# panagiotou23/model-predictive-control

Hardware: AMD Instinct MI355X
Metric: MPC solves/sec, bicycle model N=20 nx=4 nu=2, batch=65536; 1/2/4/8 GPU (higher is better)
Workload: dtype f64

## Files before the change

### include/mpc_hip.h

```cpp
#ifndef MPC_HIP_H
#define MPC_HIP_H
#include <stdint.h>

#ifdef __cplusplus
extern "C" {
#endif

enum { MPC_MODEL_KINEMATIC = 0,
       MPC_MODEL_PACEJKA = 1 };
enum { MPC_WRAP_FLOOR = 0, MPC_WRAP_FMOD = 1, MPC_WRAP_IEEE = 2 };
enum { MPC_CONSTR_NONE = 0,
       MPC_CONSTR_STATE_SQ = 1,
       MPC_CONSTR_LANE = 2,
       MPC_CONSTR_DISCS = 3 };
enum { MPC_ST_UNKNOWN = 0, MPC_ST_CONVERGED = 1, MPC_ST_MAXTIME = 2, MPC_ST_MAXITER = 3,
       MPC_ST_NOTFINITE = 4, MPC_ST_NOPROGRESS = 5, MPC_ST_INTERRUPTED = 6 };
enum { MPC_OK = 0, MPC_E_ARG = -1, MPC_E_HIP = -2, MPC_E_ALLOC = -3, MPC_E_LIMIT = -4 };

#define MPC_NSTATS 8
#define MPC_MAX_N 64
#define MPC_NREC 64

typedef struct mpc_config {
    int32_t model;
// ... 83 lines not shown

int mpc_rhs(mpc_handle *h, int B, const double *x, const double *u, double *dx, void *stream);

int mpc_rollout(mpc_handle *h, int B, int Nsim, const double *x0, const double *U, double *X,
                void *stream);

int mpc_centerline_blocks(mpc_handle *h, const double *cl, int C, void *stream);
int mpc_set_nearest_blocks(mpc_handle *h, int on);

int mpc_stage_errors(mpc_handle *h, int B, const double *pose, const double *cl,
                     const int32_t *cl_index, double *err, int32_t *idx, void *stream);

int mpc_stage_cost(mpc_handle *h, int B, const double *x, const double *u, const double *cl,
                   const int32_t *cl_index, double *out, void *stream);

int mpc_eval_cost_grad(mpc_handle *h, int B, const double *x0, const double *cl,
                       const int32_t *cl_index, const double *U, const double *y,
                       const double *Sigma, double *psi, double *grad, double *yhat, void *stream);

int mpc_eval_cost_grad_wave(mpc_handle *h, int B, const double *x0, const double *cl,
                            const int32_t *cl_index, const double *U, const double *y,
                            const double *Sigma, double *psi, double *grad, double *yhat, void *stream);

int mpc_prox_step(mpc_handle *h, int B, const double *x, const double *grad, const double *gamma,
                  double *xhat, double *p, double *out, void *stream);

int mpc_lbfgs_apply(mpc_handle *h, int B, const double *S, const double *Y, const int32_t *idx,
                    const int32_t *full, const double *mask, double *q, int32_t *ok, void *stream);

int mpc_solve_batch(mpc_handle *h, int B, const double *x0, const double *cl,
                    const int32_t *cl_index, double *U, double *lambda, double *stats,
                    void *stream);

int mpc_solve_batch_async(mpc_handle *h, int B, const double *x0, const double *cl,
                          const int32_t *cl_index, double *U, double *lambda, double *stats,
                          void *stream);
int mpc_solve_wait(mpc_handle *h);

int mpc_closed_loop(mpc_handle *h, int B, int T, int shift, double *x, const double *cl,
                    const int32_t *cl_index, double *U, double *lambda, double *traj_x,
                    double *traj_u, int32_t *fail_count, double *stats, void *stream);

int mpc_solve_active(mpc_handle *h, int B, const int32_t *active, const double *x0, const double *cl,
                     const int32_t *cl_index, double *U, double *lambda, double *stats, int32_t *n_active,
                     void *stream);

// ... 62 lines not shown
```

### model_predictive_control_amd/_lib.py

```python
import ctypes as C
import os
import subprocess

def _default_hw_queues():
    if "GPU_MAX_HW_QUEUES" in os.environ:
        return
    try:
        import torch
        if torch.cuda.is_initialized():
            return
    except Exception:
        pass
    os.environ["GPU_MAX_HW_QUEUES"] = "16"


_default_hw_queues()

_HERE = os.path.dirname(os.path.abspath(__file__))
LIB_PATH = os.environ.get("MPC_LIB_PATH", os.path.join(_HERE, "libmpc_hip.so"))
_SRC = [os.path.join(_HERE, "csrc", f) for f in ("mpc_api.hip", "mpc_handle.hpp", "mpc_launch.hpp", "mpc_rounds.hpp",
                                                  "mpc_aux.hpp", "mpc_eval.hpp", "mpc_solver.hpp", "mpc_device.hpp",
                                                  "mpc_game.hpp", "mpc_solo.hpp", "mpc_event.hpp", "mpc_step_body.hpp",
                                                  "mpc_track.hpp", "mpc_obstacles.hpp", "mpc_traffic.hpp")]
_HDR = os.path.join(os.path.dirname(_HERE), "include", "mpc_hip.h")

MODEL_KINEMATIC, MODEL_PACEJKA = 0, 1
WRAP_FLOOR, WRAP_FMOD, WRAP_IEEE = 0, 1, 2
CONSTR_NONE, CONSTR_STATE_SQ, CONSTR_LANE, CONSTR_DISCS = 0, 1, 2, 3
NSTATS = 8
ST_CONVERGED = 1

EXPORTS = [
    "mpc_default_config", "mpc_nx", "mpc_m", "mpc_create", "mpc_destroy", "mpc_last_error",
    "mpc_rhs", "mpc_rollout", "mpc_stage_errors", "mpc_stage_cost", "mpc_eval_cost_grad", "mpc_prox_step",
    "mpc_lbfgs_apply", "mpc_solve_batch", "mpc_solve_batch_async", "mpc_solve_wait", "mpc_closed_loop", "mpc_last_solve_info",
    "mpc_last_solve_info2", "mpc_math_probe", "mpc_set_groups", "mpc_last_kernel_ms", "mpc_lane_payoff",
    "mpc_set_profile", "mpc_last_speculation", "mpc_last_kernel_profile", "mpc_set_solo_max",
    "mpc_eval_cost_grad_wave", "mpc_centerline_blocks", "mpc_set_nearest_blocks", "mpc_set_memo",
    "mpc_set_round_limit", "mpc_stream_concurrency", "mpc_last_solo_ms",
    "mpc_set_poll_timeout", "mpc_debug_spin", "mpc_debug_records", "mpc_debug_record_names", "mpc_source_hash",
    "mpc_last_lookahead", "mpc_step_lds_plan", "mpc_default_params", "mpc_set_agent_params",
    "mpc_solve_active", "mpc_trigger_eval", "mpc_closed_loop_event",
    "mpc_default_bounds", "mpc_set_agent_bounds",
    "mpc_default_constraints", "mpc_set_agent_constraints",
    "mpc_default_discs", "mpc_set_agent_discs", "mpc_discs_from_plans",
    "mpc_default_rates", "mpc_set_agent_rates",
    "mpc_default_fields", "mpc_set_agent_fields", "mpc_fields_from_plans", "mpc_closed_loop_traffic_field",
    "mpc_opponents_from_plans", "mpc_closed_loop_traffic",
    "mpc_obstacles_select", "mpc_discs_from_obstacles", "mpc_fields_from_obstacles", "mpc_closed_loop_obstacles",
    "mpc_track_init", "mpc_track_windows", "mpc_track_locate", "mpc_track_select", "mpc_closed_loop_track",
]
NREC = 64
NPARAM = 31
NBOUND = 4
NCONSTR = 19
NRATE = 4
NFIELD = 2
NFSRC = 8
NDISC = 2
SCENE_MAX = 64
CONSTR_FIELDS = {"g_off": (0, 6), "D_lb": (6, 6), "D_ub": (12, 6), "lane_halfwidth": (18, 1)}
# ... 55 lines not shown
def load():
    global _lib
    if _lib is not None:
        return _lib
    if not os.path.exists(LIB_PATH):
        raise RuntimeError(
            f"{LIB_PATH} is missing: run `python -c 'import __graft_entry__ as g; g.build()'` "
            "(the MPC hot path has no CPU fallback)")
    L = C.CDLL(LIB_PATH)
    vp, ci = C.c_void_p, C.c_int
    cp = C.POINTER(MpcConfig)
    L.mpc_default_config.argtypes = [cp, ci, ci]
    L.mpc_nx.argtypes = [cp]
    L.mpc_m.argtypes = [cp]
    L.mpc_create.argtypes = [cp, ci, C.POINTER(vp)]
    L.mpc_destroy.argtypes = [vp]
    L.mpc_last_error.restype = C.c_char_p
    L.mpc_rhs.argtypes = [vp, ci, vp, vp, vp, vp]
    L.mpc_rollout.argtypes = [vp, ci, ci, vp, vp, vp, vp]
    L.mpc_stage_errors.argtypes = [vp, ci, vp, vp, vp, vp, vp, vp]
    L.mpc_stage_cost.argtypes = [vp, ci, vp, vp, vp, vp, vp, vp]
    L.mpc_eval_cost_grad.argtypes = [vp, ci, vp, vp, vp, vp, vp, vp, vp, vp, vp, vp]
    L.mpc_eval_cost_grad_wave.argtypes = [vp, ci, vp, vp, vp, vp, vp, vp, vp, vp, vp, vp]
    L.mpc_prox_step.argtypes = [vp, ci, vp, vp, vp, vp, vp, vp, vp]
    L.mpc_lbfgs_apply.argtypes = [vp, ci, vp, vp, vp, vp, vp, vp, vp, vp]
    L.mpc_solve_batch.argtypes = [vp, ci, vp, vp, vp, vp, vp, vp, vp]
    L.mpc_solve_batch_async.argtypes = [vp, ci, vp, vp, vp, vp, vp, vp, vp]
    L.mpc_solve_wait.argtypes = [vp]
    L.mpc_closed_loop.argtypes = [vp, ci, ci, ci, vp, vp, vp, vp, vp, vp, vp, vp, vp, vp]
    L.mpc_solve_active.argtypes = [vp, ci, vp, vp, vp, vp, vp, vp, vp, C.POINTER(C.c_int32), vp]
    L.mpc_trigger_eval.argtypes = [vp, ci, vp, vp, vp, C.POINTER(C.c_double), C.c_double, ci, vp, vp, vp]
    L.mpc_closed_loop_event.argtypes = [vp, ci, ci, ci, C.POINTER(C.c_double), C.c_double, ci, vp, vp, vp, vp, vp, vp,
                                        vp, vp, vp, vp, vp, vp, vp, vp]
    tp = C.POINTER(MpcTrack)
    L.mpc_track_init.argtypes = [tp, cp, ci, ci, ci, ci, ci]
    L.mpc_track_windows.argtypes = [vp, tp, vp, vp, vp]
    L.mpc_track_locate.argtypes = [vp, tp, ci, vp, vp, vp, vp, vp]
    L.mpc_track_select.argtypes = [vp, tp, ci, vp, vp, vp, vp, vp, vp]
    L.mpc_closed_loop_track.argtypes = L.mpc_closed_loop_event.argtypes + [tp, vp]
    L.mpc_last_solve_info.argtypes = [vp, C.POINTER(C.c_int64), C.POINTER(C.c_int64),
                                      C.POINTER(C.c_int64), C.POINTER(C.c_double),
                                      C.POINTER(C.c_double)]
    L.mpc_last_solve_info2.argtypes = [vp, C.POINTER(C.c_double), C.POINTER(C.c_int64)]
    L.mpc_last_speculation.argtypes = [vp, C.POINTER(C.c_int64), C.POINTER(C.c_int64)]
    L.mpc_last_lookahead.argtypes = [vp, C.POINTER(C.c_int64), C.POINTER(C.c_int64)]
    L.mpc_default_params.argtypes = [cp, C.POINTER(C.c_double)]
# ... 289 lines not shown
```

### model_predictive_control_amd/csrc/mpc_api.hip

```cpp
#include "mpc_rounds.hpp"
#include "mpc_track.hpp"
#include "mpc_obstacles.hpp"

extern "C" const char *mpc_last_error(void) { return g_err.c_str(); }
#ifndef MPC_SOURCE_SHA256
#define MPC_SOURCE_SHA256 "unknown"
#endif
extern "C" const char *mpc_source_hash(void) { return MPC_SOURCE_SHA256; }

extern "C" int mpc_default_config(mpc_config *c, int model, int N)
{
    if (!c || N < 1 || N > MPC_MAX_N || (model != MPC_MODEL_KINEMATIC && model != MPC_MODEL_PACEJKA))
        return fail(MPC_E_ARG, "mpc_default_config: bad model or horizon");
    std::memset(c, 0, sizeof(*c));
    c->model = model; c->N = N;
    c->S = 100;
    c->nfe = 4;
    c->wrap_mode = MPC_WRAP_FLOOR;
    c->lbfgs_memory = N;
    c->max_iter = 1000;
    c->max_outer = 1000;
    c->hess_heuristic = 15;
    c->max_no_progress = 10;
    c->Ts = 0.05;
// ... 412 lines not shown
    hipLaunchKernelGGL(math_probe_kernel, grid_for(n, 256), dim3(256), 0, (hipStream_t)stream, n, op, a, b, out);
    HIPCHK(hipGetLastError());
    return MPC_OK;
}

extern "C" int mpc_stage_cost(mpc_handle *h, int B, const double *x, const double *u, const double *cl,
                              const int32_t *cl_index, double *out, void *stream)
{
    int rc = check_common(h, B, "mpc_stage_cost"); if (rc) return rc;
    if (B == 0) return MPC_OK;
    if (!x || !u || !cl || !out) return fail(MPC_E_ARG, "mpc_stage_cost: null buffer");
    rc = check_tables(h, B, "mpc_stage_cost", READS_PARAMS); if (rc) return rc;
    hipStream_t s = (hipStream_t)stream;
    with_model_table(h, h->params().idx, [&](auto MODEL, auto PA, auto... pt) {
        hipLaunchKernelGGL((stage_cost_kernel<MODEL(), PA(), decltype(pt)...>), grid_for(B, 64), dim3(64), 0, s,
                           h->dc, B, x, u, cl, cl_index, out, pt...);
    });
    HIPCHK(hipGetLastError());
    return MPC_OK;
}

static int eval_cost_grad(mpc_handle *h, int B, const double *x0, const double *cl, const int32_t *cl_index,
                          const double *U, const double *y, const double *Sigma, double *psi, double *grad,
                          double *yhat, void *stream, bool wave_path)
{
    int rc = check_common(h, B, "mpc_eval_cost_grad"); if (rc) return rc;
    if (B == 0) return MPC_OK;
    if (!x0 || !cl || !U || !psi) return fail(MPC_E_ARG, "mpc_eval_cost_grad: null buffer");
    const DevCfg &c = h->dc;
    if (c.m && (!y || !Sigma)) return fail(MPC_E_ARG, "mpc_eval_cost_grad: y and Sigma are required when m > 0");
    rc = check_tables(h, B, "mpc_eval_cost_grad", READS_PARAMS | READS_CONSTR | READS_DISCS | READS_RATES | READS_FIELDS, true); if (rc) return rc;
    rc = reserve(h, B); if (rc) return rc;
    hipStream_t s = (hipStream_t)stream;
    WorkspaceHost w = h->ws;
    w.cl = cl; w.cl_index = cl_index; w.x0 = x0; w.near = near_for(h, cl);
    w.xe = const_cast<double *>(U); w.ge = grad ? grad : h->ws.ws_ge;
    w.y = const_cast<double *>(y); w.Sig = c.m ? const_cast<double *>(Sigma) : h->ws.ws_Sig;
    w.yhe = (yhat && c.m) ? yhat : h->ws.ws_yhe;
    w.psi_direct = psi;
    w.ptab = h->params().table; w.pidx = h->params().idx;
    w.ctab = h->tab[TAB_CONSTR].table; w.cidx = h->tab[TAB_CONSTR].idx;
    w.dtab = h->tab[TAB_DISCS].table; w.didx = h->tab[TAB_DISCS].idx;
    w.rtab = h->tab[TAB_RATES].table; w.ridx = h->tab[TAB_RATES].idx;
    w.ftab = h->tab[TAB_FIELDS].table; w.fidx = h->tab[TAB_FIELDS].idx;
    if (wave_path) launch_solo_eval(h, w, s, grad ? 1 : 0);
    else launch_eval(h, w, s, nullptr, nullptr, grad ? B : 0, grad ? 0 : B);
    HIPCHK(hipGetLastError());
    return MPC_OK;
}
extern "C" int mpc_eval_cost_grad(mpc_handle *h, int B, const double *x0, const double *cl, const int32_t *cl_index, const double *U,
                                  const double *y, const double *Sigma, double *psi, double *grad, double *yhat, void *stream)
{
    return eval_cost_grad(h, B, x0, cl, cl_index, U, y, Sigma, psi, grad, yhat, stream, false);
}
extern "C" int mpc_eval_cost_grad_wave(mpc_handle *h, int B, const double *x0, const double *cl, const int32_t *cl_index, const double *U,
                                       const double *y, const double *Sigma, double *psi, double *grad, double *yhat, void *stream)
{
    return eval_cost_grad(h, B, x0, cl, cl_index, U, y, Sigma, psi, grad, yhat, stream, true);
}

extern "C" int mpc_prox_step(mpc_handle *h, int B, const double *x, const double *grad, const double *gamma,
                             double *xhat, double *p, double *out, void *stream)
{
    int rc = check_common(h, B, "mpc_prox_step"); if (rc) return rc;
    if (B == 0) return MPC_OK;
    if (!x || !grad || !gamma || !out) return fail(MPC_E_ARG, "mpc_prox_step: null buffer");
    rc = check_tables(h, B, "mpc_prox_step", READS_BOX); if (rc) return rc;
    if (const BoundTable &box = h->tab[TAB_BOX]; box.table)
        hipLaunchKernelGGL(prox_box_kernel, grid_for(B, 64), dim3(64), 0, (hipStream_t)stream, h->dc, B, x, grad, gamma, xhat, p, out,
                           BoxTab{box.table, box.idx});
    else
        hipLaunchKernelGGL(prox_kernel, grid_for(B, 64), dim3(64), 0, (hipStream_t)stream, h->dc, B, x, grad, gamma, xhat, p, out);
    HIPCHK(hipGetLastError());
    return MPC_OK;
}

extern "C" int mpc_lbfgs_apply(mpc_handle *h, int B, const double *S, const double *Y, const int32_t *idx,
                               const int32_t *full, const double *mask, double *q, int32_t *ok, void *stream)
{
    int rc = check_common(h, B, "mpc_lbfgs_apply"); if (rc) return rc;
    if (B == 0) return MPC_OK;
// ... 803 lines not shown
```

### model_predictive_control_amd/csrc/mpc_eval.hpp

```cpp
#pragma once
#include "mpc_solver.hpp"

#ifndef MPC_K1B_WAVES_PAC
#define MPC_K1B_WAVES_PAC 1
#endif
#ifndef MPC_QUAD_WAVES
#define MPC_QUAD_WAVES 2
#endif

namespace mpc {

struct SlotMap {
    int nG, nC, gpad, nblk_g, nblk;
    __device__ SlotMap(const int *counts, int nG_imm, int nC_imm)
    {
        nG = counts ? counts[0] : nG_imm;
        nC = counts ? counts[1] : nC_imm;
        gpad = (nG + 63) & ~63;
        nblk_g = gpad >> 6;
        nblk = nblk_g + ((nC + 63) >> 6);
    }
};

template <int MODEL, bool PA = false>
// ... 307 lines not shown
            double gx, gy;
            kin_gen_rk(c, uk, g ? cv[p] : 0.0, kr);
            kin_gen_increment(c, uk, g ? cph[p] : 0.0, g ? cv[p] : 0.0, kr, gx, gy);
            dx[p] = g ? gx : dx[p]; dy[p] = g ? gy : dy[p];
        }
    }
    double px = x0[0], py = x0[1], epx = 0.0, epy = 0.0;
#pragma unroll
    for (int p = 0; p < PASS; p++) {
        const int k0 = 16 * p, k1 = N < 16 * (p + 1) ? N : 16 * (p + 1);
        for (int k = k0; k < k1; k++) {
#pragma clang fp contract(off)
#pragma unroll
            for (int j = 0; j < 4; j++) {
                px = px + rdlane(dx[p], (4 * k + j) & 63);
                py = py + rdlane(dy[p], (4 * k + j) & 63);
            }
            if (lane == k) { epx = px; epy = py; }
        }
    }
    if (stage_lane) { put(lane + 1, 0, epx); put(lane + 1, 1, epy); put(lane + 1, 2, eph); put(lane + 1, 3, ev); }
}

template <bool PA = false>
__global__ void __launch_bounds__(256)
rollout_wide_kernel(const DevCfg c, const WsArg<PA> w, const int *__restrict__ lists,
                    const int *__restrict__ counts)
{
    const SlotMap sm(counts, 0, 0);
    const int lane = threadIdx.x & 63, wv = threadIdx.x >> 6;
    const int uslot = blockIdx.x * 4 + wv;
    if (uslot >= sm.nblk * 64) return;
    const bool is_g = uslot < sm.gpad;
    const int kslot = is_g ? uslot : uslot - sm.gpad;
    const bool active = kslot < (is_g ? sm.nG : sm.nC);
    const int raw = active ? (is_g ? lists : lists + w.Ls)[kslot] : -1;
    if (lane == 0) w.agent_of[uslot] = raw;
    if (!active) return;
    const int a = raw & AGENT_MASK;
    const int N = c.N, n = c.n;
    const size_t St = (size_t)w.St;
    const double *__restrict__ row = ((raw & CH2_BIT) ? w.xe2 : w.xe) + (size_t)a * n;
    const bool stage_lane = lane < N;
    const double d = stage_lane ? row[2 * lane] : 0.0, dl = stage_lane ? row[2 * lane + 1] : 0.0;
    if (stage_lane) {
        w.useq[(size_t)(2 * lane) * St + uslot] = d;
// ... 382 lines not shown
```

### model_predictive_control_amd/csrc/mpc_solo.hpp

```cpp
#pragma once
#include "mpc_eval.hpp"

namespace mpc {

constexpr int SOLO_WAVES = 1;

__host__ __device__ inline bool solo_wide(int model, int nfe) { return model == KIN && nfe == 4; }
__host__ __device__ inline bool solo_dual(int model, int nfe, int N) { return !solo_wide(model, nfe) && N <= 32; }

constexpr int LA_SLOTS = 4, LA_LANES = 16, LA_ENTRIES = 8;
__host__ __device__ inline bool solo_lookahead(int model, int nfe, int N, int m, int no_la)
{
    return model == PAC && !no_la && m == 0 && N <= LA_LANES && solo_dual(model, nfe, N);
}
struct LaSlot { const double *in; double *grad; double *psi; int live, is_g; };
__host__ __device__ inline size_t la_lds_doubles(int n) { return (size_t)LA_ENTRIES * (2 * n + 2) + LA_SLOTS * 4 + 8; }

template <int MODEL> __host__ __device__ inline size_t solo_lds_doubles(int nfe, int N, int n, int M, bool hist, bool la = false)
{
    constexpr int NX = ModelDim<MODEL>::NX, JS = JacRec<MODEL>::SIZE;
    const size_t per = (size_t)(N + 1) * NX + (size_t)(JS + 1) * N;
    return (hist ? (size_t)2 * M * n : 0) + (la ? LA_SLOTS : solo_dual(MODEL, nfe, N) ? 2 : 1) * per + (la ? la_lds_doubles(n) : 0);
}

#if MPC_DEV_STAMP == 5
struct SoloClk { long long roll = 0, recs = 0, adj = 0; };
#define SOLO_CLK_ARG , SoloClk &clk
#define SOLO_CLK(field, t) do { const long long now_ = __builtin_amdgcn_s_memrealtime(); clk.field += now_ - t; t = now_; } while (0)
#else
#define SOLO_CLK_ARG
#define SOLO_CLK(field, t) do { } while (0)
#endif
template <int MODEL, class... DS>
__device__ __forceinline__ void solo_eval(const DevCfg &c, const Workspace &w, int a, int lane, int req,
                                          double *traj, double *rec SOLO_CLK_ARG, const DS &...ds)
{
#if MPC_DEV_STAMP == 5
    long long tclk = __builtin_amdgcn_s_memrealtime();
#endif
    constexpr int NX = ModelDim<MODEL>::NX, JS = JacRec<MODEL>::SIZE;
    const int N = c.N, n = c.n;
    const bool wide = solo_wide(MODEL, c.nfe), dual = solo_dual(MODEL, c.nfe, N);
    const int half = dual ? lane >> 5 : 0, hl = dual ? lane & 31 : lane;
    const bool ch2 = half == 1;
    const bool live = !ch2 || (req & REQ_SPEC) != 0;
    const bool is_g = ch2 || (req & REQ_GRAD) != 0;
    const double *__restrict__ row = (ch2 ? w.xe2 : w.xe) + (size_t)a * n;
    const bool stage_lane = live && hl < N;
    const double d = stage_lane ? row[2 * hl] : 0.0, dl = stage_lane ? row[2 * hl + 1] : 0.0;
    double *const tj = traj + (size_t)half * ((size_t)(N + 1) * NX);
    double *const rc = rec + (size_t)half * ((size_t)(JS + 1) * N);
    double x0[NX];
#pragma unroll
    for (int i = 0; i < NX; i++) x0[i] = w.x0[(size_t)a * NX + i];
    if constexpr (MODEL == KIN) {
        if (wide) kin_wide_rollout(c, x0, d, dl, lane, [=](int k, int i, double v) { tj[k * 4 + i] = v; });
    }
    if constexpr (MODEL == PAC) {
        if (hl < 4 && live) {
            double x[NX];
#pragma unroll
            for (int i = 0; i < NX; i++) { x[i] = x0[i]; if (hl == 0) tj[i] = x0[i]; }
            for (int k = 0; k < N; k++) {
                StageInput<PAC> u;
                prep_input(c, row[2 * k], row[2 * k + 1], u);
                stage_forward_quad(c, u, x, hl);
                if (hl == 0) {
#pragma unroll
                    for (int i = 0; i < NX; i++) tj[(k + 1) * NX + i] = x[i];
                }
            }
        }
    } else if (!wide && hl == 0 && live) {
        double x[NX];
#pragma unroll
        for (int i = 0; i < NX; i++) { x[i] = x0[i]; tj[i] = x0[i]; }
        for (int k = 0; k < N; k++) {
            StageInput<MODEL> u;
            prep_input(c, row[2 * k], row[2 * k + 1], u);
// ... 11 lines not shown
        const double *__restrict__ clp = w.cl_index ? w.cl + (size_t)w.cl_index[a] * 2 * (size_t)c.S : w.cl;
        double *const r = rc + hl;
        const auto put = [=](int f, double v) { r[f * N] = v; };
        if (is_g) stage_sens_record<MODEL>(c, xs, xe, d, dl, put);
        Geom g;
        stage_geom(c, w, clp, w.cl_index ? w.cl_index[a] : 0, xe[0], xe[1], g);
        constexpr bool DA = has_tab<DiscTab, DS...>, RA = has_tab<RateTab, DS...>, FA = has_tab<FieldTab, DS...>;
        if constexpr (FA)
            stage_record<MODEL>(c, w, a, ch2, is_g, hl, xs, xe, d, dl, g, put, stage_rate_uniform(pack_get<RateTab>(ds...), a, hl, N, row),
                                stage_field_uniform(pack_get<FieldTab>(ds...), a, hl, N));
        else if constexpr (DA && RA)
            stage_record<MODEL>(c, w, a, ch2, is_g, hl, xs, xe, d, dl, g, put, stage_discs_uniform(pack_get<DiscTab>(ds...), a, hl, N),
                                stage_rate_uniform(pack_get<RateTab>(ds...), a, hl, N, row));
        else if constexpr (RA)
            stage_record<MODEL>(c, w, a, ch2, is_g, hl, xs, xe, d, dl, g, put, stage_rate_uniform(pack_get<RateTab>(ds...), a, hl, N, row));
        else if constexpr (DA) stage_record<MODEL>(c, w, a, ch2, is_g, hl, xs, xe, d, dl, g, put, stage_discs_uniform(ds..., a, hl, N));
        else
        stage_record<MODEL>(c, w, a, ch2, is_g, hl, xs, xe, d, dl, g, put);
    }
    __builtin_amdgcn_wave_barrier();
    SOLO_CLK(recs, tclk);
    if constexpr (MODEL == KIN) {
        if (hl < 4 && live) {
            double *psi_out = w.psi_direct ? w.psi_direct + a : !ch2 ? w.rec + (size_t)a * REC + R_PSIE : nullptr;
            adjoint_rec_quad_kin(c, is_g, hl, [=](int k, int f) { return rc[f * N + k]; }, psi_out,
                                 (ch2 ? w.ge2 : w.ge) + (size_t)a * n);
        }
    } else if (hl == 0 && live) adjoint_rec<MODEL>(c, w, a, ch2, is_g, [=](int k, int f) { return rc[f * N + k]; });
    SOLO_CLK(adj, tclk);
}

__device__ __forceinline__ void solo_eval_la(const DevCfg &c, const Workspace &w, int a, int lane, const LaSlot *slots,
                                             double *traj, double *rec)
{
    constexpr int NX = ModelDim<PAC>::NX, JS = JacRec<PAC>::SIZE;
    const int N = c.N;
    const int sl = lane >> 4, hl = lane & 15;
    const LaSlot d = slots[sl];
    const bool live = d.live != 0, is_g = d.is_g != 0;
    const double *__restrict__ row = d.in;
    const bool stage_lane = live && hl < N;
    const double dv = stage_lane ? row[2 * hl] : 0.0, dl = stage_lane ? row[2 * hl + 1] : 0.0;
    double *const tj = traj + (size_t)sl * ((size_t)(N + 1) * NX);
    double *const rc = rec + (size_t)sl * ((size_t)(JS + 1) * N);
    double x0[NX];
#pragma unroll
    for (int i = 0; i < NX; i++) x0[i] = w.x0[(size_t)a * NX + i];
// ... 50 lines not shown
{
    const int a = blockIdx.x * blockDim.x + threadIdx.x;
    const bool on = a < w.B && rec_int_of(w.rec[(size_t)a * REC + R_PHASE]) != PH_DONE;
    const unsigned long long bal = __ballot(on);
    const int lane = threadIdx.x & 63;
    int base = 0;
    if (lane == 0 && bal != 0ull) base = atomicAdd(&ctr[1], __popcll(bal));
    base = __builtin_amdgcn_readfirstlane(base);
    if (on) list[base + __popcll(bal & ((1ull << lane) - 1ull))] = a;
}

template <int MODEL, bool PA = false, class... CT>
__global__ void __launch_bounds__(64, 1) solo_eval_kernel(const DevCfg c_, const WsArg<PA> w, int want_grad, CT... ct)
{
    static_assert(sizeof...(CT) == 0 || PA, "the constraint form exists in the per-agent-parameter form alone");
    extern __shared__ double s_solo[];
    DevCfg cm_;
    if constexpr (PA) { cm_ = c_; agent_cfg_uniform(cm_, w.ptab, w.pidx, blockIdx.x); }
    constexpr bool DA = has_tab<DiscTab, CT...> || has_tab<RateTab, CT...>;
    if constexpr (has_tab<ConTab, CT...>) agent_con_uniform(cm_, ct..., blockIdx.x);
    const DevCfg &c = PA ? cm_ : c_;
    double *traj = s_solo;
    double *rec = traj + (size_t)(c.N + 1) * ModelDim<MODEL>::NX;
#if MPC_DEV_STAMP == 5
    SoloClk clk;
    if constexpr (DA) solo_eval<MODEL>(c, w, blockIdx.x, threadIdx.x, want_grad ? REQ_GRAD : REQ_COST, traj, rec, clk, ct...);
    else
    solo_eval<MODEL>(c, w, blockIdx.x, threadIdx.x, want_grad ? REQ_GRAD : REQ_COST, traj, rec, clk);
#else
    if constexpr (DA) solo_eval<MODEL>(c, w, blockIdx.x, threadIdx.x, want_grad ? REQ_GRAD : REQ_COST, traj, rec, ct...);
    else
    solo_eval<MODEL>(c, w, blockIdx.x, threadIdx.x, want_grad ? REQ_GRAD : REQ_COST, traj, rec);
#endif
}

template <int MC, class BOX>
__device__ __forceinline__ void solo_agent_la(const DevCfg &c, const DevCfg &cm, const Workspace &w, int a, int lane, double *hist,
                                              double *traj, double *rec, double *la_base, long long max_trips, const BOX &bx)
{
#pragma clang fp contract(off)
    const int n = c.n, par = lane & 1;
    const size_t an = (size_t)a * n;
    LaCache cache(la_base, n);
    LaSlot *slots = (LaSlot *)(la_base + (size_t)LA_ENTRIES * (2 * n + 2));
    static_assert(sizeof(LaSlot) == 4 * sizeof(double), "slot descriptor layout");
    cache.clear(lane);
    int next_e = 0;
    double la_evals = 0.0, la_hits = 0.0;
    __builtin_amdgcn_wave_barrier();
    const auto ldv = [&](const double *rowp) { return lane < n ? rowp[lane] : 0.0; };
    for (long long trip = 0; trip < max_trips; trip++) {
        const AgentIn<1> in = load_agent<1>(c, w, a, lane);
        int req = advance_agent<1, MC, true, false, BOX>(c, w, a, lane, in, hist, false, true, false, 1 << 30, bx);
        if ((req & (REQ_GRAD | REQ_COST)) == 0) break;
        double rv = w.rec[(size_t)a * REC + lane];
// ... 94 lines not shown
}

#ifndef MPC_SOLO_WPS_KIN
#define MPC_SOLO_WPS_KIN 2
#endif
template <int MODEL> struct SoloOcc { static constexpr int WPS = MODEL == KIN ? MPC_SOLO_WPS_KIN : 1; };

template <int MODEL, int NE, int MC, bool LA = false, bool PA = false, class... BT>
__global__ void __launch_bounds__(64 * SOLO_WAVES, SoloOcc<MODEL>::WPS)
solo_kernel(const DevCfg c, const WsArg<PA> w, const int *__restrict__ list, int *__restrict__ ctr,
            long long max_trips, BT... bt)
{
    constexpr bool BA = sizeof...(BT) != 0, DA = has_tab<DiscTab, BT...>, CA = has_tab<ConTab, BT...>, RA = has_tab<RateTab, BT...>;
    static_assert(!BA || PA, "the box form of the persistent kernel exists in the per-agent-parameter form alone");
    static_assert((!CA && !DA) || !LA, "the lookahead is an unconstrained problem's: it has no constraint or disc form");
    static_assert(!RA || !LA, "the rate forms run without the lookahead");
    constexpr bool FA = has_tab<FieldTab, BT...>;
    static_assert(!FA || (RA && !DA && !CA), "the field forms are <..., BoxTab, RateTab, FieldTab> alone");
    using BOX = BoxOf<BA, LaneBox>;
    using CON = ConOf<CA, RowCon>;
    extern __shared__ double s_solo[];
    const int lane = threadIdx.x & 63, wv = threadIdx.x >> 6;
    const size_t per_wave = solo_lds_doubles<MODEL>(c.nfe, c.N, c.n, c.M, MC < 0);
    const bool spec = solo_dual(MODEL, c.nfe, c.N);
    double *hist = s_solo + (size_t)wv * per_wave;
    double *traj = hist + (MC < 0 ? (size_t)2 * c.M * c.n : 0);
    double *rec = traj + (size_t)(c.N + 1) * ModelDim<MODEL>::NX;
    const int total = list ? ctr[1] : w.B;
    if constexpr (LA) {
        static_assert(!LA || (MODEL == PAC && NE == 1 && SOLO_WAVES == 1), "lookahead: Pacejka, n <= 64, one wave per workgroup");
        constexpr int NXm = ModelDim<MODEL>::NX, JSm = JacRec<MODEL>::SIZE;
        rec = traj + (size_t)LA_SLOTS * ((size_t)(c.N + 1) * NXm);
        double *la_base = rec + (size_t)LA_SLOTS * ((size_t)(JSm + 1) * c.N);
        for (;;) {
            int i = 0;
            if (lane == 0) i = atomicAdd(&ctr[0], 1);
            i = __builtin_amdgcn_readfirstlane(i);
            if (i >= total) break;
            const int a = list ? list[i] : i;
            if constexpr (BA) {
                DevCfg cm = c;
                agent_cfg_uniform(cm, w.ptab, w.pidx, a);
                solo_agent_la<MC>(c, cm, w, a, lane, hist, traj, rec, la_base, max_trips, lane_box_uniform(pack_get<BoxTab>(bt...), a, lane));
            } else if constexpr (PA) {
                DevCfg cm = c;
                agent_cfg_uniform(cm, w.ptab, w.pidx, a);
                solo_agent_la<MC>(c, cm, w, a, lane, hist, traj, rec, la_base, max_trips, CfgBox());
            } else
            solo_agent_la<MC>(c, c, w, a, lane, hist, traj, rec, la_base, max_trips, CfgBox());
        }
        return;
    }
    for (;;) {
        int i = 0;
        if (lane == 0) i = atomicAdd(&ctr[0], 1);
        i = __builtin_amdgcn_readfirstlane(i);
        if (i >= total) break;
        const int a = list ? list[i] : i;
        DevCfg cm_;
        if constexpr (PA) { cm_ = c; agent_cfg_uniform(cm_, w.ptab, w.pidx, a); }
        const DevCfg &cm = PA ? cm_ : c;
        BOX bx{};
        if constexpr (BA) bx = lane_box_uniform(pack_get<BoxTab>(bt...), a, lane);
        CON cn{};
        if constexpr (CA) {
            const ConTab &ct = pack_get<ConTab>(bt...);
            agent_con_uniform(cm_, ct.ctab, ct.cidx, a);
            cn = row_con_uniform(ct, a);
        }
#if MPC_DEV_STAMP == 5
        const long long st0 = __builtin_amdgcn_s_memrealtime();
        long long ntrip = 0, t_adv = 0;
        SoloClk clk;
#endif
        for (long long trip = 0; trip < max_trips; trip++) {
#if MPC_DEV_STAMP == 5
            const long long ta = __builtin_amdgcn_s_memrealtime();
#endif
            const AgentIn<NE> in = load_agent<NE>(c, w, a, lane);
            const int req = advance_agent<NE, MC, true, false, BOX, CON, false>(c, w, a, lane, in, hist, false, spec, false, 1 << 30, bx, cn);
            if ((req & (REQ_GRAD | REQ_COST)) == 0) break;
#if MPC_DEV_STAMP == 5
            t_adv += __builtin_amdgcn_s_memrealtime() - ta;
            if constexpr (FA) solo_eval<MODEL>(cm, w, a, lane, req, traj, rec, clk, pack_get<RateTab>(bt...), pack_get<FieldTab>(bt...));
            else if constexpr (DA && RA) solo_eval<MODEL>(cm, w, a, lane, req, traj, rec, clk, pack_get<DiscTab>(bt...), pack_get<RateTab>(bt...));
            else if constexpr (RA) solo_eval<MODEL>(cm, w, a, lane, req, traj, rec, clk, pack_get<RateTab>(bt...));
            else if constexpr (DA) solo_eval<MODEL>(cm, w, a, lane, req, traj, rec, clk, pack_get<DiscTab>(bt...));
            else
            solo_eval<MODEL>(cm, w, a, lane, req, traj, rec, clk);
            ntrip++;
#else
            if constexpr (FA) solo_eval<MODEL>(cm, w, a, lane, req, traj, rec, pack_get<RateTab>(bt...), pack_get<FieldTab>(bt...));
            else if constexpr (DA && RA) solo_eval<MODEL>(cm, w, a, lane, req, traj, rec, pack_get<DiscTab>(bt...), pack_get<RateTab>(bt...));
            else if constexpr (RA) solo_eval<MODEL>(cm, w, a, lane, req, traj, rec, pack_get<RateTab>(bt...));
            else if constexpr (DA) solo_eval<MODEL>(cm, w, a, lane, req, traj, rec, pack_get<DiscTab>(bt...));
            else
            solo_eval<MODEL>(cm, w, a, lane, req, traj, rec);
#endif
        }
#if MPC_DEV_STAMP == 5
        if (lane == 0 && i < DEV_STAMPS) {
            g_dev_stamps[4 * i] = st0; g_dev_stamps[4 * i + 1] = __builtin_amdgcn_s_memrealtime();
            g_dev_stamps[4 * i + 2] = ntrip | (t_adv << 20); g_dev_stamps[4 * i + 3] = a | (clk.roll << 20);
            if (i + 32768 < DEV_STAMPS) { g_dev_stamps[4 * (i + 32768)] = clk.recs; g_dev_stamps[4 * (i + 32768) + 1] = clk.adj; }
        }
#endif
    }
}

}
```

### model_predictive_control_amd/solver.py

```python
import collections
import ctypes as C

import torch

from . import _lib


def _ptr(t):
    return None if t is None else C.c_void_p(t.data_ptr())


EventLoopResult = collections.namedtuple(
    "EventLoopResult", "x U lam held traj_x traj_u solved solve_count failures stats")

TrackLoopResult = collections.namedtuple(
    "TrackLoopResult", EventLoopResult._fields + ("cl_index", "traj_row"))

TrafficLoopResult = collections.namedtuple(
    "TrafficLoopResult", "x U lam traj_x traj_u failures stats traj_opp traj_clear table")

ObstacleLoopResult = collections.namedtuple(
    "ObstacleLoopResult", "x U lam traj_x traj_u failures stats traj_sel traj_clear table cl_index")


# ... 294 lines not shown
        self._chk(x, (B, self.nx), "x"); self._chk(u, (B, 2), "u")
        cl = self._centerline(centerline, cl_index, B)
        out = self._empty(B)
        _lib.check(self.lib.mpc_stage_cost(self._h, B, _ptr(x), _ptr(u), _ptr(cl), _ptr(cl_index),
                                           _ptr(out), self._stream()))
        return out

    def eval_cost_grad(self, x0, centerline, U, y=None, Sigma=None, cl_index=None, want_grad=True, wave=False):
        B = x0.shape[0]
        self._chk(x0, (B, self.nx), "x0"); self._chk(U, (B, self.n), "U")
        cl = self._centerline(centerline, cl_index, B)
        if self.m:
            if y is None or Sigma is None:
                raise ValueError("y and Sigma are required when the problem has constraints")
            self._chk(y, (B, self.m), "y"); self._chk(Sigma, (B, self.m), "Sigma")
        psi = self._empty(B)
        grad = self._empty(B, self.n) if want_grad else None
        yhat = self._empty(B, self.m) if self.m else None
        fn = self.lib.mpc_eval_cost_grad_wave if wave else self.lib.mpc_eval_cost_grad
        _lib.check(fn(self._h, B, _ptr(x0), _ptr(cl), _ptr(cl_index), _ptr(U), _ptr(y), _ptr(Sigma), _ptr(psi),
                      _ptr(grad), _ptr(yhat), self._stream()))
        return psi, grad, yhat

    def prox_step(self, x, grad, gamma):
        B = x.shape[0]
        self._chk(x, (B, self.n), "x"); self._chk(grad, (B, self.n), "grad"); self._chk(gamma, (B,), "gamma")
        xhat, p, out = self._empty(B, self.n), self._empty(B, self.n), self._empty(B, 2)
        _lib.check(self.lib.mpc_prox_step(self._h, B, _ptr(x), _ptr(grad), _ptr(gamma), _ptr(xhat),
                                          _ptr(p), _ptr(out), self._stream()))
        return xhat, p, out

    def lbfgs_apply(self, S, Y, idx, full, mask, q):
        B = q.shape[0]
        self._chk(S, (B, self.M, self.n), "S"); self._chk(Y, (B, self.M, self.n), "Y")
        self._chk(idx, (B,), "idx", torch.int32); self._chk(full, (B,), "full", torch.int32)
        self._chk(mask, (B, self.n), "mask"); self._chk(q, (B, self.n), "q")
        if B and (int(idx.min()) < 0 or int(idx.max()) >= self.M):
            raise ValueError("idx out of range")
        qo = q.clone()
        ok = self._empty(B, dtype=torch.int32)
        _lib.check(self.lib.mpc_lbfgs_apply(self._h, B, _ptr(S), _ptr(Y), _ptr(idx), _ptr(full), _ptr(mask),
                                            _ptr(qo), _ptr(ok), self._stream()))
        return qo, ok

    def solve(self, x0, centerline, U, lam=None, cl_index=None, inplace=False):
        B = x0.shape[0]
# ... 487 lines not shown
```

Measured before the change: 506,500.

## Split wide kinematic rollout into two half-wave candidates for speculative gradient evaluation

Adds a half-wave variant of the wide kinematic rollout, so one 64-lane wave evaluates two control candidates (the current iterate and a speculative one) at once, 32 lanes each. The solo solver now turns on speculation for the kinematic nfe=4 model and places the second candidate's trajectory and records either in a second LDS block or, when it fits, in the L-BFGS history area. History prefetch is disabled so that area can be reused. This aims to fill idle lanes and cut the number of sequential evaluation trips, at the cost of more LDS per wave, some extra per-stage work and a different order of floating-point accumulation.

```diff
diff --git a/include/mpc_hip.h b/include/mpc_hip.h
--- a/include/mpc_hip.h
+++ b/include/mpc_hip.h
@@ -129,6 +129,10 @@
                             const int32_t *cl_index, const double *U, const double *y,
                             const double *Sigma, double *psi, double *grad, double *yhat, void *stream);
 
+int mpc_eval_cost_grad_wave2(mpc_handle *h, int B, const double *x0, const double *cl,
+                             const int32_t *cl_index, const double *U, const double *U2, const double *y,
+                             const double *Sigma, double *psi, double *grad, double *grad2, double *yhat, void *stream);
+
 int mpc_prox_step(mpc_handle *h, int B, const double *x, const double *grad, const double *gamma,
                   double *xhat, double *p, double *out, void *stream);
 
diff --git a/model_predictive_control_amd/_lib.py b/model_predictive_control_amd/_lib.py
--- a/model_predictive_control_amd/_lib.py
+++ b/model_predictive_control_amd/_lib.py
@@ -36,7 +36,7 @@
     "mpc_lbfgs_apply", "mpc_solve_batch", "mpc_solve_batch_async", "mpc_solve_wait", "mpc_closed_loop", "mpc_last_solve_info",
     "mpc_last_solve_info2", "mpc_math_probe", "mpc_set_groups", "mpc_last_kernel_ms", "mpc_lane_payoff",
     "mpc_set_profile", "mpc_last_speculation", "mpc_last_kernel_profile", "mpc_set_solo_max",
-    "mpc_eval_cost_grad_wave", "mpc_centerline_blocks", "mpc_set_nearest_blocks", "mpc_set_memo",
+    "mpc_eval_cost_grad_wave", "mpc_eval_cost_grad_wave2", "mpc_centerline_blocks", "mpc_set_nearest_blocks", "mpc_set_memo",
     "mpc_set_round_limit", "mpc_stream_concurrency", "mpc_last_solo_ms",
     "mpc_set_poll_timeout", "mpc_debug_spin", "mpc_debug_records", "mpc_debug_record_names", "mpc_source_hash",
     "mpc_last_lookahead", "mpc_step_lds_plan", "mpc_default_params", "mpc_set_agent_params",
@@ -138,6 +138,7 @@
     L.mpc_stage_cost.argtypes = [vp, ci, vp, vp, vp, vp, vp, vp]
     L.mpc_eval_cost_grad.argtypes = [vp, ci, vp, vp, vp, vp, vp, vp, vp, vp, vp, vp]
     L.mpc_eval_cost_grad_wave.argtypes = [vp, ci, vp, vp, vp, vp, vp, vp, vp, vp, vp, vp]
+    L.mpc_eval_cost_grad_wave2.argtypes = [vp, ci, vp, vp, vp, vp, vp, vp, vp, vp, vp, vp, vp, vp]
     L.mpc_prox_step.argtypes = [vp, ci, vp, vp, vp, vp, vp, vp, vp]
     L.mpc_lbfgs_apply.argtypes = [vp, ci, vp, vp, vp, vp, vp, vp, vp, vp]
     L.mpc_solve_batch.argtypes = [vp, ci, vp, vp, vp, vp, vp, vp, vp]
diff --git a/model_predictive_control_amd/csrc/mpc_api.hip b/model_predictive_control_amd/csrc/mpc_api.hip
--- a/model_predictive_control_amd/csrc/mpc_api.hip
+++ b/model_predictive_control_amd/csrc/mpc_api.hip
@@ -458,7 +458,7 @@
 
 static int eval_cost_grad(mpc_handle *h, int B, const double *x0, const double *cl, const int32_t *cl_index,
                           const double *U, const double *y, const double *Sigma, double *psi, double *grad,
-                          double *yhat, void *stream, bool wave_path)
+                          double *yhat, void *stream, bool wave_path, const double *U2 = nullptr, double *grad2 = nullptr)
 {
     int rc = check_common(h, B, "mpc_eval_cost_grad"); if (rc) return rc;
     if (B == 0) return MPC_OK;
@@ -474,12 +474,13 @@
     w.y = const_cast<double *>(y); w.Sig = c.m ? const_cast<double *>(Sigma) : h->ws.ws_Sig;
     w.yhe = (yhat && c.m) ? yhat : h->ws.ws_yhe;
     w.psi_direct = psi;
+    if (U2) { w.xe2 = const_cast<double *>(U2); w.ge2 = grad2; }
     w.ptab = h->params().table; w.pidx = h->params().idx;
     w.ctab = h->tab[TAB_CONSTR].table; w.cidx = h->tab[TAB_CONSTR].idx;
     w.dtab = h->tab[TAB_DISCS].table; w.didx = h->tab[TAB_DISCS].idx;
     w.rtab = h->tab[TAB_RATES].table; w.ridx = h->tab[TAB_RATES].idx;
     w.ftab = h->tab[TAB_FIELDS].table; w.fidx = h->tab[TAB_FIELDS].idx;
-    if (wave_path) launch_solo_eval(h, w, s, grad ? 1 : 0);
+    if (wave_path) launch_solo_eval(h, w, s, (grad ? 1 : 0) | (U2 ? 2 : 0));
     else launch_eval(h, w, s, nullptr, nullptr, grad ? B : 0, grad ? 0 : B);
     HIPCHK(hipGetLastError());
     return MPC_OK;
@@ -493,6 +494,18 @@
                                        const double *y, const double *Sigma, double *psi, double *grad, double *yhat, void *stream)
 {
     return eval_cost_grad(h, B, x0, cl, cl_index, U, y, Sigma, psi, grad, yhat, stream, true);
+}
+
+extern "C" int mpc_eval_cost_grad_wave2(mpc_handle *h, int B, const double *x0, const double *cl, const int32_t *cl_index, const double *U,
+                                        const double *U2, const double *y, const double *Sigma, double *psi, double *grad, double *grad2,
+                                        double *yhat, void *stream)
+{
+    int rc = check_common(h, B, "mpc_eval_cost_grad_wave2"); if (rc) return rc;
+    if (B == 0) return MPC_OK;
+    if (!U2 || !grad2) return fail(MPC_E_ARG, "mpc_eval_cost_grad_wave2: null buffer");
+    if (!solo_halves(h->dc.model, h->dc.nfe, h->dc.N))
+        return fail(MPC_E_ARG, "mpc_eval_cost_grad_wave2: the kinematic model with nfe = 4 and N <= 32 (the half-wave form of the wide rollout)");
+    return eval_cost_grad(h, B, x0, cl, cl_index, U, y, Sigma, psi, grad, yhat, stream, true, U2, grad2);
 }
 
 extern "C" int mpc_prox_step(mpc_handle *h, int B, const double *x, const double *grad, const double *gamma,
diff --git a/model_predictive_control_amd/csrc/mpc_eval.hpp b/model_predictive_control_amd/csrc/mpc_eval.hpp
--- a/model_predictive_control_amd/csrc/mpc_eval.hpp
+++ b/model_predictive_control_amd/csrc/mpc_eval.hpp
@@ -353,6 +353,97 @@
     if (stage_lane) { put(lane + 1, 0, epx); put(lane + 1, 1, epy); put(lane + 1, 2, eph); put(lane + 1, 3, ev); }
 }
 
+__device__ __forceinline__ void kin_wide_rollout2(const DevCfg &c, const double (&x0)[4], double d, double dl, int lane,
+                                                  double *xch, double *tj)
+{
+    const int N = c.N, hl = lane & 31;
+    const bool stage_lane = hl < N, hi = lane >= 32;
+    StageInput<KIN> u;
+    prep_input(c, d, dl, u);
+    double *const uin = xch, *const inc = xch + 3 * N;
+    if (stage_lane) { uin[3 * hl] = u.ad; uin[3 * hl + 1] = u.beta; uin[3 * hl + 2] = u.sb_lr; }
+    if (hl == 0) {
+#pragma unroll
+        for (int i = 0; i < 4; i++) tj[i] = x0[i];
+    }
+    __builtin_amdgcn_wave_barrier();
+    double ph = x0[2], v = x0[3];
+    constexpr int PASS = 4;
+    double cph[PASS] = {0.0, 0.0, 0.0, 0.0}, cv[PASS] = {0.0, 0.0, 0.0, 0.0}, eph = 0.0, ev = 0.0;
+    int gen = 0;
+    bool anygen = false;
+    double n_ad = uin[0], n_beta = uin[1], n_sb = uin[2];
+#pragma unroll
+    for (int p = 0; p < PASS; p++) {
+        const int k1 = N < 8 * (p + 1) ? N : 8 * (p + 1);
+        for (int k = 8 * p; k < k1; k++) {
+            StageInput<KIN> uk;
+            uk.ad = n_ad; uk.beta = n_beta; uk.sb_lr = n_sb;
+            const int kn = k + 1 < N ? k + 1 : k;
+            n_ad = uin[3 * kn]; n_beta = uin[3 * kn + 1]; n_sb = uin[3 * kn + 2];
+            const double xs[4] = {0.0, 0.0, ph, v};
+            const unsigned long long bad = __ballot(!kin4_in_range(c, uk, xs));
+            const bool inr = (hi ? bad >> 32 : bad & 0xffffffffull) == 0ull;
+            anygen = anygen || bad != 0ull;
+#pragma unroll
+            for (int j = 0; j < 4; j++) {
+                if (hl == ((4 * k + j) & 31)) { cph[p] = ph; cv[p] = v; gen |= inr ? 0 : 1 << p; }
+                KinRK kr;
+                if (__builtin_expect(bad == 0ull, 1)) { kin_rk(c, uk, v, kr); kin_next(c, kr, ph, v); }
+                else {
+                    double pha = ph, va = v;
+                    kin_rk(c, uk, v, kr); kin_next(c, kr, pha, va);
+                    kin_gen_rk(c, uk, v, kr); kin_gen_next(c, kr, ph, v);
+                    ph = inr ? pha : ph; v = inr ? va : v;
+                }
+            }
+            if (hl == k) { eph = ph; ev = v; }
+        }
+    }
+#pragma unroll
+    for (int p = 0; p < PASS; p++) {
+        const int s = 32 * p + hl;
+        if (32 * p >= 4 * N) break;
+        const bool on = (s >> 2) < N;
+        const int k = on ? (s >> 2) : N - 1;
+        StageInput<KIN> uk;
+        uk.ad = uin[3 * k]; uk.beta = uin[3 * k + 1]; uk.sb_lr = uin[3 * k + 2];
+        const bool g = ((gen >> p) & 1) != 0 && on;
+        KinRK kr;
+        double dx, dy;
+        kin_rk(c, uk, cv[p], kr);
+        kin_increment(c, uk, cph[p], kr, !g, dx, dy);
+        if (anygen) {
+            double gx, gy;
+            kin_gen_rk(c, uk, g ? cv[p] : 0.0, kr);
+            kin_gen_increment(c, uk, g ? cph[p] : 0.0, g ? cv[p] : 0.0, kr, gx, gy);
+            dx = g ? gx : dx; dy = g ? gy : dy;
+        }
+        if (on) { inc[2 * s] = dx; inc[2 * s + 1] = dy; }
+    }
+    __builtin_amdgcn_wave_barrier();
+    double px = x0[0], py = x0[1], epx = 0.0, epy = 0.0;
+    double nx[4], ny[4];
+#pragma unroll
+    for (int j = 0; j < 4; j++) { nx[j] = inc[2 * j]; ny[j] = inc[2 * j + 1]; }
+    for (int k = 0; k < N; k++) {
+#pragma clang fp contract(off)
+        double ix[4], iy[4];
+        const int kn = k + 1 < N ? k + 1 : k;
+#pragma unroll
+        for (int j = 0; j < 4; j++) { ix[j] = nx[j]; iy[j] = ny[j]; }
+#pragma unroll
+        for (int j = 0; j < 4; j++) { nx[j] = inc[2 * (4 * kn + j)]; ny[j] = inc[2 * (4 * kn + j) + 1]; }
+#pragma unroll
+        for (int j = 0; j < 4; j++) {
+            px = px + ix[j];
+            py = py + iy[j];
+        }
+        if (hl == k) { epx = px; epy = py; }
+    }
+    if (stage_lane) { tj[(hl + 1) * 4] = epx; tj[(hl + 1) * 4 + 1] = epy; tj[(hl + 1) * 4 + 2] = eph; tj[(hl + 1) * 4 + 3] = ev; }
+}
+
 template <bool PA = false>
 __global__ void __launch_bounds__(256)
 rollout_wide_kernel(const DevCfg c, const WsArg<PA> w, const int *__restrict__ lists,
diff --git a/model_predictive_control_amd/csrc/mpc_solo.hpp b/model_predictive_control_amd/csrc/mpc_solo.hpp
--- a/model_predictive_control_amd/csrc/mpc_solo.hpp
+++ b/model_predictive_control_amd/csrc/mpc_solo.hpp
@@ -7,6 +7,7 @@
 
 __host__ __device__ inline bool solo_wide(int model, int nfe) { return model == KIN && nfe == 4; }
 __host__ __device__ inline bool solo_dual(int model, int nfe, int N) { return !solo_wide(model, nfe) && N <= 32; }
+__host__ __device__ inline bool solo_halves(int model, int nfe, int N) { return solo_wide(model, nfe) && N <= 32; }
 
 constexpr int LA_SLOTS = 4, LA_LANES = 16, LA_ENTRIES = 8;
 __host__ __device__ inline bool solo_lookahead(int model, int nfe, int N, int m, int no_la)
@@ -16,11 +17,17 @@
 struct LaSlot { const double *in; double *grad; double *psi; int live, is_g; };
 __host__ __device__ inline size_t la_lds_doubles(int n) { return (size_t)LA_ENTRIES * (2 * n + 2) + LA_SLOTS * 4 + 8; }
 
+constexpr bool SOLO_HIST_PREFETCH = false;
+template <int MODEL> __host__ __device__ inline bool solo_second_on_hist(int N, int n, int M, bool hist)
+{
+    return !SOLO_HIST_PREFETCH && hist && (size_t)2 * M * n >= (size_t)(N + 1) * ModelDim<MODEL>::NX + (size_t)(JacRec<MODEL>::SIZE + 1) * N;
+}
 template <int MODEL> __host__ __device__ inline size_t solo_lds_doubles(int nfe, int N, int n, int M, bool hist, bool la = false)
 {
     constexpr int NX = ModelDim<MODEL>::NX, JS = JacRec<MODEL>::SIZE;
     const size_t per = (size_t)(N + 1) * NX + (size_t)(JS + 1) * N;
-    return (hist ? (size_t)2 * M * n : 0) + (la ? LA_SLOTS : solo_dual(MODEL, nfe, N) ? 2 : 1) * per + (la ? la_lds_doubles(n) : 0);
+    const bool second = solo_halves(MODEL, nfe, N) && !solo_second_on_hist<MODEL>(N, n, M, hist);
+    return (hist ? (size_t)2 * M * n : 0) + (la ? LA_SLOTS : solo_dual(MODEL, nfe, N) || second ? 2 : 1) * per + (la ? la_lds_doubles(n) : 0);
 }
 
 #if MPC_DEV_STAMP == 5
@@ -33,14 +40,16 @@
 #endif
 template <int MODEL, class... DS>
 __device__ __forceinline__ void solo_eval(const DevCfg &c, const Workspace &w, int a, int lane, int req,
-                                          double *traj, double *rec SOLO_CLK_ARG, const DS &...ds)
+                                          double *traj, double *rec, double *alt SOLO_CLK_ARG, const DS &...ds)
 {
 #if MPC_DEV_STAMP == 5
     long long tclk = __builtin_amdgcn_s_memrealtime();
 #endif
     constexpr int NX = ModelDim<MODEL>::NX, JS = JacRec<MODEL>::SIZE;
     const int N = c.N, n = c.n;
-    const bool wide = solo_wide(MODEL, c.nfe), dual = solo_dual(MODEL, c.nfe, N);
+    const bool wide = solo_wide(MODEL, c.nfe);
+    const bool halves = solo_halves(MODEL, c.nfe, N) && (req & REQ_SPEC) != 0;
+    const bool dual = solo_dual(MODEL, c.nfe, N) || halves;
     const int half = dual ? lane >> 5 : 0, hl = dual ? lane & 31 : lane;
     const bool ch2 = half == 1;
     const bool live = !ch2 || (req & REQ_SPEC) != 0;
@@ -48,13 +57,17 @@
     const double *__restrict__ row = (ch2 ? w.xe2 : w.xe) + (size_t)a * n;
     const bool stage_lane = live && hl < N;
     const double d = stage_lane ? row[2 * hl] : 0.0, dl = stage_lane ? row[2 * hl + 1] : 0.0;
-    double *const tj = traj + (size_t)half * ((size_t)(N + 1) * NX);
-    double *const rc = rec + (size_t)half * ((size_t)(JS + 1) * N);
+    double *const tj = half && alt ? alt : traj + (size_t)half * ((size_t)(N + 1) * NX);
+    double *const rc = half && alt ? alt + (size_t)(N + 1) * NX : rec + (size_t)half * ((size_t)(JS + 1) * N);
     double x0[NX];
 #pragma unroll
     for (int i = 0; i < NX; i++) x0[i] = w.x0[(size_t)a * NX + i];
     if constexpr (MODEL == KIN) {
-        if (wide) kin_wide_rollout(c, x0, d, dl, lane, [=](int k, int i, double v) { tj[k * 4 + i] = v; });
+        static_assert(11 <= JS + 1, "kin_wide_rollout2's exchange area fits a record block");
+        DevCfg cr = c;
+        asm volatile("" : "+s"(cr.h), "+s"(cr.friction), "+s"(cr.N), "+s"(cr.lf), "+s"(cr.lr));
+        if (halves) kin_wide_rollout2(cr, x0, d, dl, lane, rc, tj);
+        else if (wide) kin_wide_rollout(cr, x0, d, dl, lane, [=](int k, int i, double v) { tj[k * 4 + i] = v; });
     }
     if constexpr (MODEL == PAC) {
         if (hl < 4 && live) {
@@ -112,7 +125,7 @@
     SOLO_CLK(recs, tclk);
     if constexpr (MODEL == KIN) {
         if (hl < 4 && live) {
-            double *psi_out = w.psi_direct ? w.psi_direct + a : !ch2 ? w.rec + (size_t)a * REC + R_PSIE : nullptr;
+            double *psi_out = ch2 ? nullptr : w.psi_direct ? w.psi_direct + a : w.rec + (size_t)a * REC + R_PSIE;
             adjoint_rec_quad_kin(c, is_g, hl, [=](int k, int f) { return rc[f * N + k]; }, psi_out,
                                  (ch2 ? w.ge2 : w.ge) + (size_t)a * n);
         }
@@ -209,15 +222,18 @@
     const DevCfg &c = PA ? cm_ : c_;
     double *traj = s_solo;
     double *rec = traj + (size_t)(c.N + 1) * ModelDim<MODEL>::NX;
+    double *alt = nullptr;
+    if (solo_halves(MODEL, c.nfe, c.N)) alt = rec + (size_t)(JacRec<MODEL>::SIZE + 1) * c.N;
+    const int ereq = ((want_grad & 1) ? REQ_GRAD : REQ_COST) | ((want_grad & 2) ? REQ_SPEC : 0);
 #if MPC_DEV_STAMP == 5
     SoloClk clk;
-    if constexpr (DA) solo_eval<MODEL>(c, w, blockIdx.x, threadIdx.x, want_grad ? REQ_GRAD : REQ_COST, traj, rec, clk, ct...);
+    if constexpr (DA) solo_eval<MODEL>(c, w, blockIdx.x, threadIdx.x, ereq, traj, rec, alt, clk, ct...);
     else
-    solo_eval<MODEL>(c, w, blockIdx.x, threadIdx.x, want_grad ? REQ_GRAD : REQ_COST, traj, rec, clk);
+    solo_eval<MODEL>(c, w, blockIdx.x, threadIdx.x, ereq, traj, rec, alt, clk);
 #else
-    if constexpr (DA) solo_eval<MODEL>(c, w, blockIdx.x, threadIdx.x, want_grad ? REQ_GRAD : REQ_COST, traj, rec, ct...);
+    if constexpr (DA) solo_eval<MODEL>(c, w, blockIdx.x, threadIdx.x, ereq, traj, rec, alt, ct...);
     else
-    solo_eval<MODEL>(c, w, blockIdx.x, threadIdx.x, want_grad ? REQ_GRAD : REQ_COST, traj, rec);
+    solo_eval<MODEL>(c, w, blockIdx.x, threadIdx.x, ereq, traj, rec, alt);
 #endif
 }
 
@@ -358,10 +374,13 @@
     extern __shared__ double s_solo[];
     const int lane = threadIdx.x & 63, wv = threadIdx.x >> 6;
     const size_t per_wave = solo_lds_doubles<MODEL>(c.nfe, c.N, c.n, c.M, MC < 0);
-    const bool spec = solo_dual(MODEL, c.nfe, c.N);
+    const bool spec = solo_dual(MODEL, c.nfe, c.N) || solo_halves(MODEL, c.nfe, c.N);
     double *hist = s_solo + (size_t)wv * per_wave;
     double *traj = hist + (MC < 0 ? (size_t)2 * c.M * c.n : 0);
     double *rec = traj + (size_t)(c.N + 1) * ModelDim<MODEL>::NX;
+    double *alt = nullptr;
+    if (solo_halves(MODEL, c.nfe, c.N))
+        alt = solo_second_on_hist<MODEL>(c.N, c.n, c.M, MC < 0) ? hist : rec + (size_t)(JacRec<MODEL>::SIZE + 1) * c.N;
     const int total = list ? ctr[1] : w.B;
     if constexpr (LA) {
         static_assert(!LA || (MODEL == PAC && NE == 1 && SOLO_WAVES == 1), "lookahead: Pacejka, n <= 64, one wave per workgroup");
@@ -406,7 +425,7 @@
         }
 #if MPC_DEV_STAMP == 5
         const long long st0 = __builtin_amdgcn_s_memrealtime();
-        long long ntrip = 0, t_adv = 0;
+        long long ntrip = 0, t_adv = 0, nhess = 0;
         SoloClk clk;
 #endif
         for (long long trip = 0; trip < max_trips; trip++) {
@@ -414,34 +433,35 @@
             const long long ta = __builtin_amdgcn_s_memrealtime();
 #endif
             const AgentIn<NE> in = load_agent<NE>(c, w, a, lane);
-            const int req = advance_agent<NE, MC, true, false, BOX, CON, false>(c, w, a, lane, in, hist, false, spec, false, 1 << 30, bx, cn);
+            const int req = advance_agent<NE, MC, true, false, BOX, CON, false>(c, w, a, lane, in, hist, SOLO_HIST_PREFETCH, spec, false, 1 << 30, bx, cn);
             if ((req & (REQ_GRAD | REQ_COST)) == 0) break;
 #if MPC_DEV_STAMP == 5
             t_adv += __builtin_amdgcn_s_memrealtime() - ta;
-            if constexpr (FA) solo_eval<MODEL>(cm, w, a, lane, req, traj, rec, clk, pack_get<RateTab>(bt...), pack_get<FieldTab>(bt...));
-            else if constexpr (DA && RA) solo_eval<MODEL>(cm, w, a, lane, req, traj, rec, clk, pack_get<DiscTab>(bt...), pack_get<RateTab>(bt...));
-            else if constexpr (RA) solo_eval<MODEL>(cm, w, a, lane, req, traj, rec, clk, pack_get<RateTab>(bt...));
-            else if constexpr (DA) solo_eval<MODEL>(cm, w, a, lane, req, traj, rec, clk, pack_get<DiscTab>(bt...));
+            if ((req & (REQ_GRAD | REQ_COST | REQ_SPEC)) == REQ_GRAD && (rec_int_of(w.rec[(size_t)a * REC + R_PHASE]) & PH_MASK) == PH_W_HESS) nhess++;
+            if constexpr (FA) solo_eval<MODEL>(cm, w, a, lane, req, traj, rec, alt, clk, pack_get<RateTab>(bt...), pack_get<FieldTab>(bt...));
+            else if constexpr (DA && RA) solo_eval<MODEL>(cm, w, a, lane, req, traj, rec, alt, clk, pack_get<DiscTab>(bt...), pack_get<RateTab>(bt...));
+            else if constexpr (RA) solo_eval<MODEL>(cm, w, a, lane, req, traj, rec, alt, clk, pack_get<RateTab>(bt...));
+            else if constexpr (DA) solo_eval<MODEL>(cm, w, a, lane, req, traj, rec, alt, clk, pack_get<DiscTab>(bt...));
             else
-            solo_eval<MODEL>(cm, w, a, lane, req, traj, rec, clk);
+            solo_eval<MODEL>(cm, w, a, lane, req, traj, rec, alt, clk);
             ntrip++;
 #else
-            if constexpr (FA) solo_eval<MODEL>(cm, w, a, lane, req, traj, rec, pack_get<RateTab>(bt...), pack_get<FieldTab>(bt...));
-            else if constexpr (DA && RA) solo_eval<MODEL>(cm, w, a, lane, req, traj, rec, pack_get<DiscTab>(bt...), pack_get<RateTab>(bt...));
-            else if constexpr (RA) solo_eval<MODEL>(cm, w, a, lane, req, traj, rec, pack_get<RateTab>(bt...));
-            else if constexpr (DA) solo_eval<MODEL>(cm, w, a, lane, req, traj, rec, pack_get<DiscTab>(bt...));
+            if constexpr (FA) solo_eval<MODEL>(cm, w, a, lane, req, traj, rec, alt, pack_get<RateTab>(bt...), pack_get<FieldTab>(bt...));
+            else if constexpr (DA && RA) solo_eval<MODEL>(cm, w, a, lane, req, traj, rec, alt, pack_get<DiscTab>(bt...), pack_get<RateTab>(bt...));
+            else if constexpr (RA) solo_eval<MODEL>(cm, w, a, lane, req, traj, rec, alt, pack_get<RateTab>(bt...));
+            else if constexpr (DA) solo_eval<MODEL>(cm, w, a, lane, req, traj, rec, alt, pack_get<DiscTab>(bt...));
             else
-            solo_eval<MODEL>(cm, w, a, lane, req, traj, rec);
+            solo_eval<MODEL>(cm, w, a, lane, req, traj, rec, alt);
 #endif
         }
 #if MPC_DEV_STAMP == 5
         if (lane == 0 && i < DEV_STAMPS) {
             g_dev_stamps[4 * i] = st0; g_dev_stamps[4 * i + 1] = __builtin_amdgcn_s_memrealtime();
             g_dev_stamps[4 * i + 2] = ntrip | (t_adv << 20); g_dev_stamps[4 * i + 3] = a | (clk.roll << 20);
-            if (i + 32768 < DEV_STAMPS) { g_dev_stamps[4 * (i + 32768)] = clk.recs; g_dev_stamps[4 * (i + 32768) + 1] = clk.adj; }
-        }
-#endif
-    }
-}
-
-}
+            if (i + 32768 < DEV_STAMPS) { g_dev_stamps[4 * (i + 32768)] = clk.recs; g_dev_stamps[4 * (i + 32768) + 1] = clk.adj; g_dev_stamps[4 * (i + 32768) + 2] = nhess; }
+        }
+#endif
+    }
+}
+
+}
diff --git a/model_predictive_control_amd/solver.py b/model_predictive_control_amd/solver.py
--- a/model_predictive_control_amd/solver.py
+++ b/model_predictive_control_amd/solver.py
@@ -340,6 +340,22 @@
                       _ptr(grad), _ptr(yhat), self._stream()))
         return psi, grad, yhat
 
+    def eval_cost_grad_pair(self, x0, centerline, U, U2, y=None, Sigma=None, cl_index=None, want_grad=True):
+        B = x0.shape[0]
+        self._chk(x0, (B, self.nx), "x0"); self._chk(U, (B, self.n), "U"); self._chk(U2, (B, self.n), "U2")
+        cl = self._centerline(centerline, cl_index, B)
+        if self.m:
+            if y is None or Sigma is None:
+                raise ValueError("y and Sigma are required when the problem has constraints")
+            self._chk(y, (B, self.m), "y"); self._chk(Sigma, (B, self.m), "Sigma")
+        psi = self._empty(B)
+        grad = self._empty(B, self.n) if want_grad else None
+        grad2 = self._empty(B, self.n)
+        yhat = self._empty(B, self.m) if self.m else None
+        _lib.check(self.lib.mpc_eval_cost_grad_wave2(self._h, B, _ptr(x0), _ptr(cl), _ptr(cl_index), _ptr(U), _ptr(U2), _ptr(y),
+                                                     _ptr(Sigma), _ptr(psi), _ptr(grad), _ptr(grad2), _ptr(yhat), self._stream()))
+        return psi, grad, grad2, yhat
+
     def prox_step(self, x, grad, gamma):
         B = x.shape[0]
         self._chk(x, (B, self.n), "x"); self._chk(grad, (B, self.n), "grad"); self._chk(gamma, (B,), "gamma")
```

New measurement: 512,400, median of 6. 1.2% higher.
